# tum-vision/pnec

Hardware: AMD Instinct MI355X
Metric: PNEC pose solves/sec (512 corr, 10 GN iters) (higher is better)
Workload: dtype f64; 1 GPU; configs[1]: batch of 100k simulated frame pairs x 512 anisotropic-covariance correspondences per GPU; pairs_total=100000, launcher=single process, residual=PNEC target frame, setup_launches_before_warmup=15, pairs_per_gpu=100000, correspondences=512

## Files before the change

pnec_amd/csrc/pnec_solve_kernel.hpp:

```cpp
#pragma once

#include <type_traits>

#include "pnec_device.hpp"


#define PNEC_FOR_EACH_GEOMETRY(X) \
  X(1, 1, 0) X(2, 1, 0) X(4, 1, 0) X(4, 2, 0) X(4, 4, 0) X(4, 8, 0) \
  X(8, 1, 3) X(12, 1, 3) X(8, 2, 3) X(8, 4, 3) X(8, 8, 3) X(8, 1, 0) X(1, 8, 0)
#define PNEC_FOR_EACH_AOS_GEOMETRY(X) \
  X(1, 1, 0) X(2, 1, 0) X(4, 1, 0) X(4, 4, 0) X(4, 8, 0) X(8, 1, 3) X(8, 2, 3) X(8, 4, 3) X(8, 8, 3) X(8, 1, 0)
constexpr int kStreamWaves = 8;

namespace pnec_hip {

struct SolveArgs {
  const double *data;
  const int64_t *block_offset;
  const int32_t *count;
  const int32_t *pair_index;
  const double *init_q;
  const double *init_t;
  const double *hyp_t;
  double *out_q;
  double *out_t;
  double *out_cost;
  int32_t *out_iterations;
  int32_t *out_status;
  unsigned long long *trace;
  unsigned long long *work;
  int64_t n_solves;
  int32_t n_hyp;
  int32_t numeric_jacobian;
  const double *aos_bvs1, *aos_bvs2, *aos_covs, *aos_covs_host;
  const int64_t *aos_offsets;
  unsigned long long *done_counter;
  unsigned long long *host_flag;
  unsigned long long flag_value, n_blocks_total;
  double reg;
  double inv_max_radius;
  double inv_min_radius;
  pnec_hip_options opt;
};
inline void finish_args(SolveArgs &a) {
  a.inv_max_radius = 1.0 / a.opt.max_trust_region_radius;
  a.inv_min_radius = 1.0 / a.opt.min_trust_region_radius;
}

__device__ __forceinline__ int64_t xcd_contiguous_index(int64_t b, int64_t n) {
  const int64_t xcd = b & 7, q = n >> 3, r = n & 7;
  const int64_t base = (xcd < r) ? xcd * (q + 1) : r * (q + 1) + (xcd - r) * q;
  return base + (b >> 3);
}

enum : int {
  kQ = 0,
  kTheta = 4,
  kPhi = 5,
  kCost = 6,
  kXNorm = 7,
  kInvRadius = 8,
  kDec = 9,
  kModel = 10,
  kQc = 11,
  kThetaC = 15,
  kPhiC = 16,
  kDiag = 17,
  kScaleSq = 22,
  kInvScaleSq = 27,
  kGmax = 32,
  kSumsFinite = 33,
  kSums = 36,
  kTcur = 84,
  kSlab = 88
};
constexpr int kUnif = 18;
enum : int { kIIter = 0, kIFirst, kIReuseDiag, kINumInvalid, kIStepOk,
              kILast,
              kIPark,
              kITerm,
              kINumI = 8 };

__host__ __device__ constexpr bool geometry_ok(int mode, int cpl, int wpp, int ldsk) {
  const int nc = num_components(mode);
  if (cpl == 12) return wpp == 1 && ldsk == 3 && nc <= 12;
  const long lds = (long)wpp * (ldsk * nc * kWave * 8 + (kSlab + kUnif) * 8 + kINumI * 4) + (wpp > 1 ? 2L * wpp * kSumSlots * 8 : 0);
  if (lds > 160 * 1024) return false;
  if (cpl == 8 && ldsk == 0) return nc <= 18;
  return nc * (cpl - ldsk) <= 72;
}


__device__ __forceinline__ double atan2_c(double y, double x) {
  if (y == 0.0) return copysign(signbit(x) ? 3.14159265358979311600e+00 : 0.0, y);
  return atan2_lean(y, x);
}
__device__ __forceinline__ void start_angles(double x, double y, double z, double &theta, double &phi) {
  const double n = sqrt(x * x + y * y + z * z);
  if (n == 0.0) {
    theta = 0.0;
    phi = 0.0;
    return;
  }
  theta = acos_lean(z / n);
  phi = (fabs(theta) < 1e-10) ? 0.0 : atan2_c(y / n, x / n);
}

template <int CPL, int REGK>
__host__ __device__ constexpr int slot_corr(int k, int lane) {
  if (CPL == 1) return lane;
  if (k < (REGK & ~1)) return 2 * kWave * (k / 2) + 2 * lane + (k & 1);
  return kWave * k + lane;
}

template <int NC, int CPL, int REGK>
__device__ __forceinline__ void load_resident(const double *__restrict__ base, int n, int stride,
                                              int first_corr, int lane, double (&d)[REGK][NC],
                                              double *lds ) {
  (void)n;
  if constexpr (CPL == 1) {
    const int idx = first_corr + lane;
    const bool in = idx < stride;
#pragma unroll
    for (int c = 0; c < NC; ++c) d[0][c] = in ? base[(int64_t)c * stride + idx] : 0.0;
  } else {
    using pair_t = __attribute__((ext_vector_type(2))) double;
    auto load_pair = [&](auto jc) {
      constexpr int j = decltype(jc)::value;
      const int idx = first_corr + 2 * kWave * j + 2 * lane;
      const bool in = idx < stride;
#pragma unroll
      for (int c = 0; c < NC; ++c) {
        pair_t v = {0.0, 0.0};
        if (in) v = *reinterpret_cast<const pair_t *>(base + (int64_t)c * stride + idx);
        d[2 * j][c] = v.x;
        d[2 * j + 1][c] = v.y;
      }
    };
    if constexpr (REGK >= 2) load_pair(std::integral_constant<int, 0>{});
    if constexpr (REGK >= 4) load_pair(std::integral_constant<int, 1>{});
    if constexpr (REGK >= 6) load_pair(std::integral_constant<int, 2>{});
    if constexpr (REGK >= 8) load_pair(std::integral_constant<int, 3>{});
    if constexpr (REGK & 1) {
      const int idx = first_corr + kWave * (REGK - 1) + lane;
      const bool in = idx < stride;
#pragma unroll
      for (int c = 0; c < NC; ++c) d[REGK - 1][c] = in ? base[(int64_t)c * stride + idx] : 0.0;
    }
    typedef __attribute__((address_space(3))) void lds_void;
    typedef const __attribute__((address_space(1))) void global_void;
#pragma unroll
    for (int k = REGK; k < CPL; ++k) {
      const int chunk = first_corr + kWave * k;
      if (chunk < stride) {
        if (lane < kWave / 2) {
#pragma unroll
          for (int c = 0; c < NC; ++c)
            __builtin_amdgcn_global_load_lds((global_void *)(base + (int64_t)c * stride + chunk + 2 * lane),
                                             (lds_void *)(uintptr_t)(uint32_t)(uintptr_t)(lds + ((k - REGK) * NC + c) * kWave),
                                             16, 0, 0);
        }
      } else {
#pragma unroll
        for (int c = 0; c < NC; ++c) lds[((k - REGK) * NC + c) * kWave + lane] = 0.0;
      }
    }
  }
}

template <int NC, int CPL, int REGK>
__device__ __forceinline__ void load_resident_aos(const double *__restrict__ b1, const double *__restrict__ b2,
                                                  const double *__restrict__ cv, const double *__restrict__ ch,
                                                  int n, int first_corr, int lane, double (&d)[REGK][NC],
                                                  double *lds ) {
  auto put = [&](auto kc, int c, double v) {
    constexpr int k = decltype(kc)::value;
    if constexpr (k < REGK) d[k][c] = v;
    else lds[((k - REGK) * NC + c) * kWave + lane] = v;
  };
  auto load_slot = [&](auto kc) {
    constexpr int k = decltype(kc)::value;
    const int idx = first_corr + slot_corr<CPL, REGK>(k, lane);
    const bool in = idx < n;
    const int64_t j = in ? idx : 0;
#pragma unroll
    for (int c = 0; c < 3; ++c) {
      put(kc, c, in ? b1[3 * j + c] : 0.0);
      put(kc, 3 + c, in ? b2[3 * j + c] : 0.0);
    }
    if constexpr (NC >= 12) {
      const double *C = cv + 9 * j;
      put(kc, 6, in ? C[0] : 0.0);
      put(kc, 7, in ? 0.5 * (C[1] + C[3]) : 0.0);
      put(kc, 8, in ? 0.5 * (C[2] + C[6]) : 0.0);
      put(kc, 9, in ? C[4] : 0.0);
      put(kc, 10, in ? 0.5 * (C[5] + C[7]) : 0.0);
      put(kc, 11, in ? C[8] : 0.0);
    }
    if constexpr (NC >= 18) {
      const double *C = ch + 9 * j;
      put(kc, 12, in ? C[0] : 0.0);
      put(kc, 13, in ? 0.5 * (C[1] + C[3]) : 0.0);
      put(kc, 14, in ? 0.5 * (C[2] + C[6]) : 0.0);
      put(kc, 15, in ? C[4] : 0.0);
      put(kc, 16, in ? 0.5 * (C[5] + C[7]) : 0.0);
      put(kc, 17, in ? C[8] : 0.0);
    }
  };
  load_slot(std::integral_constant<int, 0>{});
  if constexpr (CPL >= 2) load_slot(std::integral_constant<int, 1>{});
  if constexpr (CPL >= 4) {
    load_slot(std::integral_constant<int, 2>{});
    load_slot(std::integral_constant<int, 3>{});
  }
  if constexpr (CPL >= 8) {
    load_slot(std::integral_constant<int, 4>{});
    load_slot(std::integral_constant<int, 5>{});
    load_slot(std::integral_constant<int, 6>{});
    load_slot(std::integral_constant<int, 7>{});
  }
}

template <int MODE, int REGK, int LDSK>
__device__ __forceinline__ void pass_resident(const double (&d)[REGK][num_components(MODE)],
                                              const double *lds , int nslots,
                                              int lane, const PassUniforms &U, double reg,
                                              double (&acc)[kNumAcc]) {
  constexpr int NC = num_components(MODE);
  auto eval_slot = [&](auto kc) {
    constexpr int k = decltype(kc)::value;
    double r, J[5];
    eval_corr<MODE>(d[k], U, reg, r, J);
    accumulate(r, J, acc);
  };
  eval_slot(std::integral_constant<int, 0>{});
  if constexpr (REGK > 1) eval_slot(std::integral_constant<int, 1>{});
  if constexpr (REGK > 2) {
    if (nslots > 2) {
      eval_slot(std::integral_constant<int, 2>{});
      if constexpr (REGK > 3) eval_slot(std::integral_constant<int, 3>{});
      if constexpr (REGK > 4) eval_slot(std::integral_constant<int, 4>{});
      if constexpr (REGK > 5) eval_slot(std::integral_constant<int, 5>{});
      if constexpr (REGK > 6) eval_slot(std::integral_constant<int, 6>{});
      if constexpr (REGK > 7) eval_slot(std::integral_constant<int, 7>{});
    }
  }
#pragma unroll
  for (int k = 0; k < LDSK; ++k) {
    if (REGK + k >= nslots) continue;
    double e[NC];
#pragma unroll
    for (int c = 0; c < NC; ++c) e[c] = lds[(k * NC + c) * kWave + lane];
    double r, J[5];
    eval_corr<MODE>(e, U, reg, r, J);
    accumulate(r, J, acc);
  }
}

template <int MODE, int REGK, int LDSK>
__device__ __forceinline__ void pass_cost_resident(const double (&d)[REGK][num_components(MODE)],
                                                   const double *lds , int nslots,
                                                   int lane, const PassUniforms &U, double reg,
                                                   double &acc0, double &z) {
  constexpr int NC = num_components(MODE);
  auto eval_slot = [&](auto kc) {
    constexpr int k = decltype(kc)::value;
    double r, kk;
    eval_cost<MODE>(d[k], U, reg, r, kk);
    acc0 = __builtin_fma(r, r, acc0);
    z = __builtin_fma(kk, 0.0, z);
  };
  eval_slot(std::integral_constant<int, 0>{});
  if constexpr (REGK > 1) eval_slot(std::integral_constant<int, 1>{});
  if constexpr (REGK > 2) {
    if (nslots > 2) {
      eval_slot(std::integral_constant<int, 2>{});
      if constexpr (REGK > 3) eval_slot(std::integral_constant<int, 3>{});
      if constexpr (REGK > 4) eval_slot(std::integral_constant<int, 4>{});
      if constexpr (REGK > 5) eval_slot(std::integral_constant<int, 5>{});
      if constexpr (REGK > 6) eval_slot(std::integral_constant<int, 6>{});
      if constexpr (REGK > 7) eval_slot(std::integral_constant<int, 7>{});
    }
  }
#pragma unroll
  for (int k = 0; k < LDSK; ++k) {
    if (REGK + k >= nslots) continue;
    double e[NC];
#pragma unroll
    for (int c = 0; c < NC; ++c) e[c] = lds[(k * NC + c) * kWave + lane];
    double r, kk;
    eval_cost<MODE>(e, U, reg, r, kk);
    acc0 = __builtin_fma(r, r, acc0);
    z = __builtin_fma(kk, 0.0, z);
  }
}

__device__ __forceinline__ void pose_uniforms_sc(double st, double ct, double sp, double cp, const double (&q)[4],
                                                 double *u) {
  double R[9];
  rot_from_quat(q, R);
#pragma unroll
  for (int i = 0; i < 9; ++i) u[i] = R[i];
  u[9] = st * cp;   u[10] = st * sp;  u[11] = ct;
  u[12] = ct * cp;  u[13] = ct * sp;  u[14] = -st;
}
__device__ __forceinline__ void pose_uniforms(double theta, double phi, const double (&q)[4], double *u) {
  double st, ct, sp, cp;
  sincos_bounded(theta, st, ct);
  sincos_bounded(phi, sp, cp);
  pose_uniforms_sc(st, ct, sp, cp, q, u);
}

__device__ __forceinline__ void write_result(const SolveArgs &a, int64_t s, const double *slab, int iteration,
                                             int term) {
  const double q0 = slab[kQ + 0], q1 = slab[kQ + 1], q2 = slab[kQ + 2], q3 = slab[kQ + 3];
  const double qn = fast_rsqrt(q0 * q0 + q1 * q1 + q2 * q2 + q3 * q3);
  if (a.out_q) {
    a.out_q[4 * s + 0] = q0 * qn;
    a.out_q[4 * s + 1] = q1 * qn;
    a.out_q[4 * s + 2] = q2 * qn;
    a.out_q[4 * s + 3] = q3 * qn;
  }
  if (a.out_t) {
    a.out_t[3 * s + 0] = slab[kTcur + 0];
    a.out_t[3 * s + 1] = slab[kTcur + 1];
    a.out_t[3 * s + 2] = slab[kTcur + 2];
  }
  if (a.out_cost) a.out_cost[s] = slab[kCost];
  if (a.out_iterations) a.out_iterations[s] = iteration;
  if (a.out_status) a.out_status[s] = term;
}

template <bool COST_FIRST>
__device__ __forceinline__ int lm_advance(double *slab, int *ist, double *unif, const pnec_hip_options &o,
                                          double inv_max_radius, double inv_min_radius) {
  int iteration = ist[kIIter], reuse_diagonal = ist[kIReuseDiag];
  int num_invalid = ist[kINumInvalid], step_ok = ist[kIStepOk];
  const int first = ist[kIFirst];
  const int pass_kind = ist[kILast];
  const bool last = pass_kind == 1;
  const bool cost_first = COST_FIRST && pass_kind == 2;
  int park = ist[kIPark];
  int term = -1;

  double S[kNumAcc];
  const double *cand_sums = slab + kSums + (park ^ 1) * kSumSlots;
#pragma unroll
  for (int j = 0; j < kNumAcc; ++j) S[j] = cand_sums[sum_slot(j)];
  const bool rest_ok = slab[kSumsFinite] != 0.0;
  const double qc0 = slab[kQc + 0], qc1 = slab[kQc + 1], qc2 = slab[kQc + 2], qc3 = slab[kQc + 3];
  const double thc0 = slab[kThetaC], phc0 = slab[kPhiC];
  const double cost = slab[kCost], model = slab[kModel], xnorm = slab[kXNorm];
  double inv_radius = slab[kInvRadius], dec = slab[kDec], gmax = slab[kGmax];
  double x[6];

  double cost_c = 0.5 * S[0];
  const bool cost_ok = finite_d(cost_c);
  bool accept = false;
  double rho = 0.0;
  if (first) {
    if (!(cost_ok && rest_ok)) {
      slab[kQ + 0] = qc0; slab[kQ + 1] = qc1; slab[kQ + 2] = qc2; slab[kQ + 3] = qc3;
      slab[kTheta] = thc0;
      slab[kPhi] = phc0;
        slab[kTcur + 0] = unif[9]; slab[kTcur + 1] = unif[10]; slab[kTcur + 2] = unif[11];
      slab[kCost] = cost_c;
      term = PNEC_HIP_TERM_BAD_INITIAL;
    } else {
#pragma unroll
      for (int i = 0; i < 5; ++i) {
        const double f = (i >= 2) ? 2.0 : 1.0, inv_f = (i >= 2) ? 0.5 : 1.0;
        const double hii = S[6 + tri(i, i)] * (f * f);
        const double a = (o.jacobi_scaling ? 1.0 + fast_sqrt(hii) : 1.0) * inv_f;
        slab[kInvScaleSq + i] = a * a;
        slab[kScaleSq + i] = fast_rcp(a * a);
      }
      accept = true;
    }
  } else {
    if (!cost_ok) cost_c = 1.7976931348623157e308;
    if (o.check_convergence) {
#pragma unroll
      for (int k = 0; k < 4; ++k) x[k] = slab[kQ + k];
      x[4] = slab[kTheta];
      x[5] = slab[kPhi];
      double dn = (x[4] - thc0) * (x[4] - thc0) + (x[5] - phc0) * (x[5] - phc0);
      dn = __builtin_fma(x[0] - qc0, x[0] - qc0, dn);
      dn = __builtin_fma(x[1] - qc1, x[1] - qc1, dn);
      dn = __builtin_fma(x[2] - qc2, x[2] - qc2, dn);
      dn = __builtin_fma(x[3] - qc3, x[3] - qc3, dn);
      const double step_norm = fast_sqrt(dn);
      if (step_norm <= o.parameter_tolerance * (xnorm + o.parameter_tolerance))
        term = PNEC_HIP_TERM_PARAMETER_TOL;
      else if (fabs(cost - cost_c) <= o.function_tolerance * cost)
        term = PNEC_HIP_TERM_FUNCTION_TOL;
    }
    if (term < 0) {
      rho = (cost - cost_c) * fast_rcp(model);
      accept = rho > o.min_relative_decrease;
      if (accept && !rest_ok) term = PNEC_HIP_TERM_BAD_INITIAL;
    }
  }

  if (term < 0 && cost_first && accept) {
    ist[kILast] = 0;
    return -1;
  }
  if (term < 0 && last) {
    if (accept) {
      slab[kQ + 0] = qc0; slab[kQ + 1] = qc1; slab[kQ + 2] = qc2; slab[kQ + 3] = qc3;
      slab[kTheta] = thc0;
      slab[kPhi] = phc0;
        slab[kTcur + 0] = unif[9]; slab[kTcur + 1] = unif[10]; slab[kTcur + 2] = unif[11];
      slab[kCost] = cost_c;
    }
    term = PNEC_HIP_TERM_MAX_ITERATIONS;
  }
  if (term < 0) {
    double H[15], g[5], diag[5];
    if (accept) {
      x[0] = qc0; x[1] = qc1; x[2] = qc2; x[3] = qc3; x[4] = thc0; x[5] = phc0;
#pragma unroll
      for (int i = 0; i < 5; ++i) g[i] = S[1 + i];
#pragma unroll
      for (int i = 0; i < 15; ++i) H[i] = S[6 + i];
      if (o.check_convergence) {
        gmax = 0.0;
#pragma unroll
        for (int i = 0; i < 5; ++i) gmax = fmax(gmax, fabs(g[i]) * ((i >= 2) ? 2.0 : 1.0));
      }
      if (first) {
        inv_radius = fast_rcp(o.initial_trust_region_radius);
      } else {
        const double c1 = 2.0 * rho - 1.0;
        inv_radius = fmax(inv_max_radius, inv_radius * fmax(1.0 / 3.0, 1.0 - c1 * c1 * c1));
      }
      dec = 2.0;
      park ^= 1;
      step_ok = 1;
      reuse_diagonal = 0;
#pragma unroll
      for (int k = 0; k < 4; ++k) slab[kQ + k] = x[k];
      slab[kTheta] = x[4];
      slab[kPhi] = x[5];
        slab[kTcur + 0] = unif[9]; slab[kTcur + 1] = unif[10]; slab[kTcur + 2] = unif[11];
      slab[kCost] = cost_c;
      if (o.check_convergence) {
        slab[kXNorm] = fast_sqrt(x[4] * x[4] + x[5] * x[5] + x[0] * x[0] + x[1] * x[1] + x[2] * x[2] + x[3] * x[3]);
        slab[kGmax] = gmax;
      }
    } else {
#pragma unroll
      for (int k = 0; k < 4; ++k) x[k] = slab[kQ + k];
      x[4] = slab[kTheta];
      x[5] = slab[kPhi];
      const double *cur_sums = slab + kSums + park * kSumSlots;
#pragma unroll
      for (int i = 0; i < 5; ++i) g[i] = cur_sums[sum_slot(1 + i)];
#pragma unroll
      for (int i = 0; i < 15; ++i) H[i] = cur_sums[sum_slot(6 + i)];
      inv_radius = inv_radius * dec;
      dec = 2.0 * dec;
      reuse_diagonal = 1;
    }
    if (reuse_diagonal) {
#pragma unroll
      for (int i = 0; i < 5; ++i) diag[i] = slab[kDiag + i];
    }

    for (bool retry = false;; retry = true) {
      if (iteration >= o.max_num_iterations) { term = PNEC_HIP_TERM_MAX_ITERATIONS; break; }
      if (retry) {
        const double *cur_sums = slab + kSums + park * kSumSlots;
#pragma unroll
        for (int i = 0; i < 15; ++i) H[i] = cur_sums[sum_slot(6 + i)];
      }
      if (o.check_convergence && step_ok && gmax <= o.gradient_tolerance) {
        term = PNEC_HIP_TERM_GRADIENT_TOL; break;
      }
      if (inv_radius > inv_min_radius) { term = PNEC_HIP_TERM_MIN_RADIUS; break; }
      ++iteration;
      step_ok = 0;

      if (!reuse_diagonal) {
#pragma unroll
        for (int i = 0; i < 5; ++i) {
          diag[i] = fmin(fmax(H[tri(i, i)] * slab[kScaleSq + i], o.min_lm_diagonal), o.max_lm_diagonal) *
                    slab[kInvScaleSq + i];
          slab[kDiag + i] = diag[i];
        }
      }
      double dr[5], y[5], step[5];
#pragma unroll
      for (int i = 0; i < 5; ++i) {
        dr[i] = diag[i] * inv_radius;
        H[tri(i, i)] += dr[i];
      }
      bool valid = chol_solve5(H, g, y);
      double sg = 0.0, sd = 0.0;
#pragma unroll
      for (int i = 0; i < 5; ++i) {
        step[i] = -y[i];
        sg = __builtin_fma(step[i], g[i], sg);
        sd = __builtin_fma(dr[i] * step[i], step[i], sd);
      }
      const double model_change = 0.5 * (sd - sg);
      valid = valid && (model_change > 0.0);
      if (!valid) {
        if (++num_invalid >= o.max_num_consecutive_invalid_steps) { term = PNEC_HIP_TERM_INVALID_STEPS; break; }
        inv_radius = 2.0 * inv_radius;
        reuse_diagonal = 1;
        continue;
      }
      num_invalid = 0;

      const double dx = 0.5 * step[2], dy = 0.5 * step[3], dz = 0.5 * step[4];
      const double thc = x[4] + step[0];
      const double phc = x[5] + step[1];
      const double nd2 = dx * dx + dy * dy + dz * dz;
      const double ind = nd2 > 0.0 ? fast_rsqrt(nd2) : 0.0, nd = nd2 * ind;
      const int role = (int)(threadIdx.x & 3);
      const double angle = role == 0 ? nd : (role == 1 ? thc : phc);
      double sa, ca;
      sincos_bounded_pinned(angle, sa, ca);
      const double sn = quad_broadcast<0>(sa), aw = quad_broadcast<0>(ca);
      const double st = quad_broadcast<1>(sa), ct = quad_broadcast<1>(ca);
      const double sp = quad_broadcast<2>(sa), cp = quad_broadcast<2>(ca);
      const double sbd = sn * ind;
      const double ax = sbd * dx, ay = sbd * dy, az = sbd * dz;
      double qc[4];
      qc[0] = aw * x[0] + ax * x[3] + ay * x[2] - az * x[1];
      qc[1] = aw * x[1] - ax * x[2] + ay * x[3] + az * x[0];
      qc[2] = aw * x[2] + ax * x[1] - ay * x[0] + az * x[3];
      qc[3] = aw * x[3] - ax * x[0] - ay * x[1] - az * x[2];
      pose_uniforms_sc(st, ct, sp, cp, qc, unif);
#pragma unroll
      for (int k = 0; k < 4; ++k) slab[kQc + k] = qc[k];
      slab[kThetaC] = thc;
      slab[kPhiC] = phc;
      slab[kModel] = model_change;
      const double cost_now = accept ? cost_c : cost;
      ist[kILast] = iteration >= o.max_num_iterations ? 1 : ((COST_FIRST && (!accept || model_change <= 4.0e-15 * cost_now)) ? 2 : 0);
      break;
    }
    slab[kInvRadius] = inv_radius;
    slab[kDec] = dec;
  }
  ist[kIPark] = park;

  ist[kIIter] = iteration;
  ist[kIFirst] = (term < 0 || !first) ? 0 : 1;
  ist[kIReuseDiag] = reuse_diagonal;
  ist[kINumInvalid] = num_invalid;
  ist[kIStepOk] = step_ok;
  return term;
}

constexpr int kNumPoses = 12;
__device__ __forceinline__ void numeric_poses(const double *slab, int lane, double (*nu)[12], double *inv2h) {
  if (lane < kNumPoses) {
    const int prm = lane >> 1;
    double x[6] = {slab[kThetaC], slab[kPhiC], slab[kQc + 0], slab[kQc + 1], slab[kQc + 2], slab[kQc + 3]};
    const double xv = prm == 0 ? x[0] : (prm == 1 ? x[1] : (prm == 2 ? x[2] : (prm == 3 ? x[3] : (prm == 4 ? x[4] : x[5]))));
    const double h = fmax(1.4901161193847656e-08, fabs(xv) * 1e-6);
    const double xp = (lane & 1) ? xv - h : xv + h;
#pragma unroll
    for (int k = 0; k < 6; ++k) x[k] = (k == prm) ? xp : x[k];
    double u[kUnif];
    const double q[4] = {x[2], x[3], x[4], x[5]};
    pose_uniforms(x[0], x[1], q, u);
#pragma unroll
    for (int i = 0; i < 12; ++i) nu[lane][i] = u[i];
    if ((lane & 1) == 0) inv2h[prm] = 1.0 / h / 2.0;
  }
}
template <int MODE>
__device__ __forceinline__ void eval_corr_numeric(const double (&e)[num_components(MODE)], const PassUniforms &U,
                                                  const double (*nu)[12], const double *inv2h, const double *qc,
                                                  double reg, double &r, double (&J)[5]) {
  double kk;
  eval_cost<MODE>(e, U, reg, r, kk);
  double Ja[6];
#pragma unroll 1
  for (int prm = 0; prm < 6; ++prm) {
    double rr[2];
#pragma unroll
    for (int sgn = 0; sgn < 2; ++sgn) {
      PassUniforms V;
      const double *u = nu[2 * prm + sgn];
#pragma unroll
      for (int i = 0; i < 9; ++i) V.R[i] = u[i];
#pragma unroll
      for (int i = 0; i < 3; ++i) V.t[i] = u[9 + i];
      eval_cost<MODE>(e, V, reg, rr[sgn], kk);
    }
    Ja[prm] = (rr[0] - rr[1]) * inv2h[prm];
  }
  J[0] = Ja[0];
  J[1] = Ja[1];
  const double qx = qc[0], qy = qc[1], qz = qc[2], qw = qc[3];
  J[2] = 0.5 * (Ja[2] * qw + Ja[3] * -qz + Ja[4] * qy + Ja[5] * -qx);
  J[3] = 0.5 * (Ja[2] * qz + Ja[3] * qw + Ja[4] * -qx + Ja[5] * -qy);
  J[4] = 0.5 * (Ja[2] * -qy + Ja[3] * qx + Ja[4] * qw + Ja[5] * -qz);
}

#ifdef PNEC_ISA_MARKS
#define PNEC_MARK(name) asm volatile("; PNEC_MARK " name)
#else
#define PNEC_MARK(name)
#endif

constexpr int SRC_PLANES = 0;
constexpr int SRC_AOS = 1;
template <int MODE, int CPL, int WPP, int LDSK, bool RESIDENT, int SRC = SRC_PLANES>
__global__ __launch_bounds__(kWave *WPP, (CPL == 8 && LDSK == 0) ? 1 : 2) void lm_solve_kernel(const SolveArgs a) {
  static_assert(SRC != SRC_AOS || RESIDENT, "the AoS source is only built for the on-chip-resident geometries");
  constexpr int NC = num_components(MODE);
  constexpr int RCPL = CPL > 8 ? 8 : CPL;
  constexpr int TAILK = CPL - RCPL;
  static_assert(TAILK == 0 || (TAILK == 4 && WPP == 1 && RESIDENT && SRC != SRC_AOS), "the tail form is (12, 1, 3) on the batch's planes");
  constexpr int REGK = RESIDENT ? RCPL - LDSK : 1;
  const int lane = threadIdx.x & (kWave - 1);
  const int wave = threadIdx.x >> 6;
  const int64_t slot = xcd_contiguous_index(blockIdx.x, a.n_solves);
  const int64_t pair = a.pair_index ? (int64_t)a.pair_index[slot / a.n_hyp] : slot / a.n_hyp;
  const int64_t s = pair * a.n_hyp + slot % a.n_hyp;
  const double *__restrict__ base = nullptr;
  int n;
  int64_t aos0 = 0;
  if constexpr (SRC == SRC_AOS) {
    aos0 = a.aos_offsets[pair];
    n = (int)(a.aos_offsets[pair + 1] - aos0);
  } else {
    base = a.data + a.block_offset[pair];
    n = a.count[pair];
  }
  const int stride = (n + kWave - 1) & ~(kWave - 1);
  const pnec_hip_options &o = a.opt;
  const double reg = a.reg;

  unsigned long long t_begin = 0, t_loaded = 0;
  if (a.trace) t_begin = __builtin_amdgcn_s_memtime();

  __shared__ double slab_all[WPP][kSlab];
  __shared__ double unif_all[WPP][kUnif];
  __shared__ int ist_all[WPP][kINumI];
  [[maybe_unused]] __shared__ double xw[2][WPP > 1 ? WPP : 1][kSumSlots];
  [[maybe_unused]] __shared__ double nunif[RESIDENT ? 1 : kNumPoses][12];
  [[maybe_unused]] __shared__ double ninv2h[8];
  [[maybe_unused]] __shared__ double ldata[LDSK > 0 ? WPP : 1][LDSK > 0 ? LDSK : 1][NC][LDSK > 0 ? kWave : 1];
  double *slab = slab_all[WPP > 1 ? 0 : wave];
  double *unif = unif_all[WPP > 1 ? 0 : wave];
  int *ist = ist_all[WPP > 1 ? 0 : wave];
  [[maybe_unused]] int parity = 0;

  double d[REGK][NC];
  if constexpr (RESIDENT && SRC == SRC_AOS)
    load_resident_aos<NC, RCPL, REGK>(a.aos_bvs1 + 3 * aos0, a.aos_bvs2 + 3 * aos0, NC >= 12 ? a.aos_covs + 9 * aos0 : nullptr,
                                     NC >= 18 ? a.aos_covs_host + 9 * aos0 : nullptr, n, wave * RCPL * kWave, lane, d,
                                     &ldata[LDSK > 0 ? wave : 0][0][0][0]);
  else if constexpr (RESIDENT)
    load_resident<NC, RCPL, REGK>(base, n, stride, wave * RCPL * kWave, lane, d, &ldata[LDSK > 0 ? wave : 0][0][0][0]);
  [[maybe_unused]] int nslots = 0;
  if constexpr (RESIDENT) {
#pragma unroll
    for (int k = 0; k < RCPL; ++k) nslots += (n > wave * RCPL * kWave + slot_corr<RCPL, REGK>(k, 0)) ? 1 : 0;
  }
  [[maybe_unused]] int ntail = 0;
  [[maybe_unused]] const char *tail_base = nullptr;
  [[maybe_unused]] size_t tail_plane_bytes = 0;
  if constexpr (TAILK > 0) {
#pragma unroll
    for (int t = 0; t < TAILK; ++t) ntail += (n > RCPL * kWave + 2 * kWave * (t / 2) + (t & 1)) ? 1 : 0;
    const unsigned long long b64 = reinterpret_cast<unsigned long long>(base) + (unsigned long long)RCPL * kWave * sizeof(double);
    const unsigned blo = (unsigned)__builtin_amdgcn_readfirstlane((int)(unsigned)b64);
    const unsigned bhi = (unsigned)__builtin_amdgcn_readfirstlane((int)(unsigned)(b64 >> 32));
    tail_base = reinterpret_cast<const char *>(((unsigned long long)bhi << 32) | blo);
    tail_plane_bytes = (size_t)(unsigned)__builtin_amdgcn_readfirstlane(stride) * sizeof(double);
    ntail = __builtin_amdgcn_readfirstlane(ntail);
  }
  if (a.trace) {
    __builtin_amdgcn_s_waitcnt(0);
    t_loaded = __builtin_amdgcn_s_memtime();
  }

  if (lane == 0 && (WPP == 1 || wave == 0)) {
    double th, ph;
    const double *t0 = a.hyp_t ? a.hyp_t + 3 * s : a.init_t + 3 * pair;
    start_angles(t0[0], t0[1], t0[2], th, ph);
    double q[4];
#pragma unroll
    for (int k = 0; k < 4; ++k) {
      q[k] = a.init_q[pair * 4 + k];
      slab[kQc + k] = q[k];
    }
    slab[kThetaC] = th;
    slab[kPhiC] = ph;
    pose_uniforms(th, ph, q, unif);
    ist[kIIter] = 0;
    ist[kIFirst] = 1;
    ist[kIReuseDiag] = 0;
    ist[kINumInvalid] = 0;
    ist[kIStepOk] = 1;
    ist[kILast] = o.max_num_iterations <= 0 ? 1 : 0;
    ist[kIPark] = 0;
  }
  const double inv_max_radius = a.inv_max_radius, inv_min_radius = a.inv_min_radius;
  if constexpr (RESIDENT && LDSK > 0 && SRC != SRC_AOS) __builtin_amdgcn_s_waitcnt(0x0F70);
  __builtin_amdgcn_fence(__ATOMIC_RELEASE, "wavefront");
  if constexpr (WPP > 1) __syncthreads();

  int term;
  int n_full_passes = 0, n_cost_passes = 0;
  for (;;) {
    PNEC_MARK("uniforms");
    {
      __builtin_amdgcn_fence(__ATOMIC_ACQUIRE, "wavefront");
      PassUniforms U;
#pragma unroll
      for (int i = 0; i < 9; ++i) U.R[i] = to_sgpr(unif[i]);
#pragma unroll
      for (int i = 0; i < 3; ++i) U.t[i] = to_sgpr(unif[9 + i]);
#pragma unroll
      for (int i = 0; i < 3; ++i) U.bth[i] = to_sgpr(unif[12 + i]);
      U.bph[0] = -U.t[1];
      U.bph[1] = U.t[0];
      U.bph[2] = 0.0;
      double c[6];
      bool cost_only = false;
      if constexpr (RESIDENT) cost_only = to_sgpr(ist[kILast]) != 0;
      n_cost_passes += cost_only ? 1 : 0;
      n_full_passes += cost_only ? 0 : 1;
      if (cost_only) {
        PNEC_MARK("pass_cost");
        if constexpr (RESIDENT) {
          double a0 = 0.0, z = 0.0;
          pass_cost_resident<MODE, REGK, LDSK>(d, &ldata[LDSK > 0 ? wave : 0][0][0][0], nslots, lane, U, reg,
                                               a0, z);
          c[0] = wave_reduce_acc0_row0(a0);
          c[1] = __builtin_amdgcn_ballot_w64(!(z == 0.0)) == 0ull ? 0.0 : __builtin_nan("");
          c[2] = c[3] = c[4] = c[5] = 0.0;
          if constexpr (TAILK > 0) {
            if (ntail > 0) {
              double a1 = 0.0, z1 = 0.0;
              const char *tb = tail_base;
              const size_t plane_bytes = tail_plane_bytes;
              const unsigned voff = 16u * (unsigned)lane;
              auto tail_cost = [&](auto tc) {
                constexpr int t = decltype(tc)::value;
                constexpr unsigned imm = 2u * kWave * 8u * (t / 2) + 8u * (t & 1);
                const bool in = RCPL * kWave + 2 * kWave * (t / 2) + 2 * lane < stride;
                double e[NC];
                load_planes_saddr<NC, (int)imm>(e, tb, plane_bytes, voff, in);
                double r, kk;
                eval_cost<MODE>(e, U, reg, r, kk);
                a1 = __builtin_fma(r, r, a1);
                z1 = __builtin_fma(kk, 0.0, z1);
              };
              tail_cost(std::integral_constant<int, 0>{});
              __builtin_amdgcn_sched_barrier(0);
              tail_cost(std::integral_constant<int, 1>{});
              __builtin_amdgcn_sched_barrier(0);
              if (ntail > 2) {
                tail_cost(std::integral_constant<int, 2>{});
                __builtin_amdgcn_sched_barrier(0);
                tail_cost(std::integral_constant<int, 3>{});
                __builtin_amdgcn_sched_barrier(0);
              }
              c[0] += wave_reduce_acc0_row0(a1);
              c[1] += __builtin_amdgcn_ballot_w64(!(z1 == 0.0)) == 0ull ? 0.0 : __builtin_nan("");
            }
          }
        }
      } else {
        double acc[kNumAcc];
#pragma unroll
        for (int j = 0; j < kNumAcc; ++j) acc[j] = 0.0;
        PNEC_MARK("pass");
        if constexpr (RESIDENT) {
          pass_resident<MODE, REGK, LDSK>(d, &ldata[LDSK > 0 ? wave : 0][0][0][0], nslots, lane, U, reg, acc);
        } else {
          const bool numeric = a.numeric_jacobian != 0;
          if (numeric) {
            if (wave == 0) numeric_poses(slab, lane, nunif, ninv2h);
            __syncthreads();
          }
          for (int idx = threadIdx.x; idx < stride; idx += kWave * WPP) {
            double e[NC];
#pragma unroll
            for (int c = 0; c < NC; ++c) e[c] = base[(int64_t)c * stride + idx];
            double r, J[5];
            if (numeric) eval_corr_numeric<MODE>(e, U, nunif, ninv2h, slab + kQc, reg, r, J);
            else eval_corr<MODE>(e, U, reg, r, J);
            accumulate(r, J, acc);
          }
        }
        PNEC_MARK("reduce");
        wave_reduce21_rows(acc, c);
        if constexpr (TAILK > 0) {
          if (ntail > 0) {
            double *park_sums = slab + kSums + (to_sgpr(ist[kIPark]) ^ 1) * kSumSlots;
            if ((lane & 15) == 0) {
#pragma unroll
              for (int i = 0; i < 6; ++i) park_sums[(lane >> 4) * 6 + i] = c[i];
            }
#pragma unroll
            for (int j = 0; j < kNumAcc; ++j) acc[j] = 0.0;
            const char *tb = tail_base;
            const size_t plane_bytes = tail_plane_bytes;
            const unsigned voff = 16u * (unsigned)lane;
            auto tail_slot = [&](auto tc) {
              constexpr int t = decltype(tc)::value;
              constexpr unsigned imm = 2u * kWave * 8u * (t / 2) + 8u * (t & 1);
              const bool in = RCPL * kWave + 2 * kWave * (t / 2) + 2 * lane < stride;
              double e[NC];
              load_planes_saddr<NC, (int)imm>(e, tb, plane_bytes, voff, in);
              double r, J[5];
              eval_corr<MODE>(e, U, reg, r, J);
              accumulate(r, J, acc);
            };
            tail_slot(std::integral_constant<int, 0>{});
            __builtin_amdgcn_sched_barrier(0);
            tail_slot(std::integral_constant<int, 1>{});
            __builtin_amdgcn_sched_barrier(0);
            if (ntail > 2) {
              tail_slot(std::integral_constant<int, 2>{});
              __builtin_amdgcn_sched_barrier(0);
              tail_slot(std::integral_constant<int, 3>{});
              __builtin_amdgcn_sched_barrier(0);
            }
            double c2[6];
            wave_reduce21_rows(acc, c2);
            __builtin_amdgcn_fence(__ATOMIC_RELEASE, "wavefront");
            __builtin_amdgcn_wave_barrier();
            __builtin_amdgcn_fence(__ATOMIC_ACQUIRE, "wavefront");
#pragma unroll
            for (int i = 0; i < 6; ++i) c[i] = park_sums[(lane >> 4) * 6 + i] + c2[i];
          }
        }
      }
      double *cand_sums = slab + kSums + (to_sgpr(ist[kIPark]) ^ 1) * kSumSlots;
      if constexpr (WPP == 1) {
        const bool fin = rows_all_finite(c);
        if ((lane & 15) == 0) {
#pragma unroll
          for (int i = 0; i < 6; ++i) cand_sums[(lane >> 4) * 6 + i] = c[i];
          if (lane == 0) slab[kSumsFinite] = fin ? 1.0 : 0.0;
        }
      } else {
        if ((lane & 15) == 0) {
#pragma unroll
          for (int i = 0; i < 6; ++i) xw[parity][wave][(lane >> 4) * 6 + i] = c[i];
        }
        __syncthreads();
        if (wave == 0 && lane == 0) {
          double z = 0.0;
#pragma unroll
          for (int j = 0; j < kSumSlots; ++j) {
            double t = xw[parity][0][j];
#pragma unroll
            for (int w = 1; w < WPP; ++w) t += xw[parity][w][j];
            cand_sums[j] = t;
            z = __builtin_fma(t, 0.0, z);
          }
          slab[kSumsFinite] = (z == 0.0) ? 1.0 : 0.0;
        }
        parity ^= 1;
      }
    }

    PNEC_MARK("advance");
    __builtin_amdgcn_fence(__ATOMIC_RELEASE, "wavefront");
    int t = -1;
    if constexpr (WPP == 1) {
      __builtin_amdgcn_s_setprio(3);
      if (lane < 4) t = lm_advance<RESIDENT>(slab, ist, unif, o, inv_max_radius, inv_min_radius);
      term = to_sgpr(t);
      __builtin_amdgcn_s_setprio(0);
      __builtin_amdgcn_fence(__ATOMIC_RELEASE, "wavefront");
    } else {
      if (wave == 0) {
        __builtin_amdgcn_s_setprio(3);
        if (lane < 4) t = lm_advance<RESIDENT>(slab, ist, unif, o, inv_max_radius, inv_min_radius);
        if (lane == 0) ist[kITerm] = t;
        __builtin_amdgcn_s_setprio(0);
      }
      __syncthreads();
      term = to_sgpr(ist[kITerm]);
    }
    if (term >= 0) break;
  }

  PNEC_MARK("result");
  if (threadIdx.x == 0) {
    write_result(a, s, slab, ist[kIIter], term);
    if (a.work) {
      atomicAdd(a.work + 0, (unsigned long long)n_full_passes * (unsigned long long)n);
      atomicAdd(a.work + 1, (unsigned long long)n_cost_passes * (unsigned long long)n);
    }
    if constexpr (SRC == SRC_AOS) {
      __threadfence_system();
      const unsigned long long done = atomicAdd(a.done_counter, 1ull) + 1ull;
      if (done == a.n_blocks_total) {
        __hip_atomic_store(a.host_flag, a.flag_value, __ATOMIC_RELEASE, __HIP_MEMORY_SCOPE_SYSTEM);
      }
    }
    if (a.trace && threadIdx.x == 0) {
      unsigned hw = 0;
      asm volatile("s_getreg_b32 %0, hwreg(HW_REG_HW_ID)" : "=s"(hw));
      unsigned xcc = 0;
      asm volatile("s_getreg_b32 %0, hwreg(HW_REG_XCC_ID)" : "=s"(xcc));
      a.trace[4 * (size_t)blockIdx.x + 0] = t_begin;
      a.trace[4 * (size_t)blockIdx.x + 1] = t_loaded;
      a.trace[4 * (size_t)blockIdx.x + 2] = __builtin_amdgcn_s_memtime();
      a.trace[4 * (size_t)blockIdx.x + 3] = ((unsigned long long)xcc << 32) | hw;
    }
  }
}

}
```

Before: 36.78 million solves/s.

## Speculate rejected-step fallback candidates in spare lanes and specialize the residual Jacobian

In single-wave resident geometries, three extra lane quads now solve the damped system at successively larger damping while the primary quad solves the normal step. The fallback candidates are staged in LDS, so a rejected step can take the next candidate directly and skip a re-solve in the serial Levenberg-Marquardt advance. A hand-written residual and Jacobian routine for the NEC and target modes replaces the generic eval_corr in the solve passes to cut arithmetic per correspondence. In exchange the change adds LDS usage, extra lanes in the advance step, and extra control logic, and it can only help when steps are actually rejected.

```diff
diff --git a/pnec_amd/csrc/pnec_solve_kernel.hpp b/pnec_amd/csrc/pnec_solve_kernel.hpp
--- a/pnec_amd/csrc/pnec_solve_kernel.hpp
+++ b/pnec_amd/csrc/pnec_solve_kernel.hpp
@@ -79,12 +79,17 @@
               kILast,
               kIPark,
               kITerm,
+              kISpec = kITerm,
               kINumI = 8 };
+constexpr int kNumFallbacks = 3;
+enum : int { kSpModel = 0, kSpQc = 1, kSpThetaC = 5, kSpPhiC = 6, kSpValid = 7, kSpUnif = 8 , kSpecSlot = 24 };
+static_assert(kQc - kModel == kSpQc && kThetaC - kModel == kSpThetaC && kPhiC - kModel == kSpPhiC, "slot layout = slab layout");
 
 __host__ __device__ constexpr bool geometry_ok(int mode, int cpl, int wpp, int ldsk) {
   const int nc = num_components(mode);
   if (cpl == 12) return wpp == 1 && ldsk == 3 && nc <= 12;
-  const long lds = (long)wpp * (ldsk * nc * kWave * 8 + (kSlab + kUnif) * 8 + kINumI * 4) + (wpp > 1 ? 2L * wpp * kSumSlots * 8 : 0);
+  const long lds = (long)wpp * (ldsk * nc * kWave * 8 + (kSlab + kUnif) * 8 + kINumI * 4) + (wpp > 1 ? 2L * wpp * kSumSlots * 8 : 0) +
+                   (wpp == 1 ? kNumFallbacks * kSpecSlot * 8 : 0);
   if (lds > 160 * 1024) return false;
   if (cpl == 8 && ldsk == 0) return nc <= 18;
   return nc * (cpl - ldsk) <= 72;
@@ -221,6 +226,52 @@
   }
 }
 
+template <int MODE>
+__device__ __forceinline__ void eval_corr_solve(const double (&d)[num_components(MODE)], const PassUniforms &U,
+                                                double reg, double &r, double (&J)[5]) {
+  if constexpr (MODE != PNEC_HIP_MODE_NEC && MODE != PNEC_HIP_MODE_TARGET) {
+    eval_corr<MODE>(d, U, reg, r, J);
+  } else {
+    const double f1x = d[0], f1y = d[1], f1z = d[2];
+    const double f2x = d[3], f2y = d[4], f2z = d[5];
+    const double *R = U.R;
+    const double mx = U.t[1] * f1z - U.t[2] * f1y;
+    const double my = U.t[2] * f1x - U.t[0] * f1z;
+    const double mz = U.t[0] * f1y - U.t[1] * f1x;
+    const double gx = R[0] * mx + R[3] * my + R[6] * mz;
+    const double gy = R[1] * mx + R[4] * my + R[7] * mz;
+    const double gz = R[2] * mx + R[5] * my + R[8] * mz;
+    const double n = f2x * gx + f2y * gy + f2z * gz;
+    double wx, wy, wz;
+    if constexpr (MODE == PNEC_HIP_MODE_NEC) {
+      r = n;
+      wx = f2x; wy = f2y; wz = f2z;
+    } else {
+      const double sgx = d[6] * gx + d[7] * gy + d[8] * gz;
+      const double sgy = d[7] * gx + d[9] * gy + d[10] * gz;
+      const double sgz = d[8] * gx + d[10] * gy + d[11] * gz;
+      const double den = gx * sgx + gy * sgy + gz * sgz + reg;
+      const double y = fast_rsqrt(fmax(den, kTinyDen));
+      r = n * y;
+      const double c = r * y;
+      wx = y * (f2x - c * sgx);
+      wy = y * (f2y - c * sgy);
+      wz = y * (f2z - c * sgz);
+    }
+    const double ux = R[0] * wx + R[1] * wy + R[2] * wz;
+    const double uy = R[3] * wx + R[4] * wy + R[5] * wz;
+    const double uz = R[6] * wx + R[7] * wy + R[8] * wz;
+    J[2] = __builtin_fma(uy, mz, -(uz * my));
+    J[3] = __builtin_fma(uz, mx, -(ux * mz));
+    J[4] = __builtin_fma(ux, my, -(uy * mx));
+    const double jx = __builtin_fma(f1y, uz, -(f1z * uy));
+    const double jy = __builtin_fma(f1z, ux, -(f1x * uz));
+    const double jz = __builtin_fma(f1x, uy, -(f1y * ux));
+    J[0] = U.bth[0] * jx + U.bth[1] * jy + U.bth[2] * jz;
+    J[1] = U.bph[0] * jx + U.bph[1] * jy;
+  }
+}
+
 template <int MODE, int REGK, int LDSK>
 __device__ __forceinline__ void pass_resident(const double (&d)[REGK][num_components(MODE)],
                                               const double *lds , int nslots,
@@ -230,7 +281,7 @@
   auto eval_slot = [&](auto kc) {
     constexpr int k = decltype(kc)::value;
     double r, J[5];
-    eval_corr<MODE>(d[k], U, reg, r, J);
+    eval_corr_solve<MODE>(d[k], U, reg, r, J);
     accumulate(r, J, acc);
   };
   eval_slot(std::integral_constant<int, 0>{});
@@ -252,7 +303,7 @@
 #pragma unroll
     for (int c = 0; c < NC; ++c) e[c] = lds[(k * NC + c) * kWave + lane];
     double r, J[5];
-    eval_corr<MODE>(e, U, reg, r, J);
+    eval_corr_solve<MODE>(e, U, reg, r, J);
     accumulate(r, J, acc);
   }
 }
@@ -331,9 +382,14 @@
   if (a.out_status) a.out_status[s] = term;
 }
 
-template <bool COST_FIRST>
+template <bool COST_FIRST, int NFB = 0>
 __device__ __forceinline__ int lm_advance(double *slab, int *ist, double *unif, const pnec_hip_options &o,
-                                          double inv_max_radius, double inv_min_radius) {
+                                          double inv_max_radius, double inv_min_radius,
+                                          [[maybe_unused]] double *spec = nullptr ) {
+  static_assert(NFB == 0 || NFB == kNumFallbacks, "one quad per fallback: lanes 4 .. 15");
+  [[maybe_unused]] const int quad = NFB > 0 ? (int)((threadIdx.x >> 2) & 3) : 0;
+  [[maybe_unused]] int served = 0;
+  if constexpr (NFB > 0) served = ist[kISpec];
   int iteration = ist[kIIter], reuse_diagonal = ist[kIReuseDiag];
   int num_invalid = ist[kINumInvalid], step_ok = ist[kIStepOk];
   const int first = ist[kIFirst];
@@ -406,6 +462,30 @@
     ist[kILast] = 0;
     return -1;
   }
+  if constexpr (NFB > 0) {
+    if (term < 0 && !last && !accept && served < NFB && iteration < o.max_num_iterations) {
+      const double *slot = spec + served * kSpecSlot;
+      if (slot[kSpValid] != 0.0) {
+        inv_radius = inv_radius * dec;
+        dec = 2.0 * dec;
+        ++iteration;
+#pragma unroll
+        for (int k = 0; k < kSpValid; ++k) slab[kModel + k] = slot[k];
+#pragma unroll
+        for (int i = 0; i < 15; ++i) unif[i] = slot[kSpUnif + i];
+        slab[kInvRadius] = inv_radius;
+        slab[kDec] = dec;
+        ist[kILast] = iteration >= o.max_num_iterations ? 1 : (COST_FIRST ? 2 : 0);
+        ist[kISpec] = served + 1;
+        ist[kIIter] = iteration;
+        ist[kIFirst] = 0;
+        ist[kIReuseDiag] = 1;
+        ist[kINumInvalid] = 0;
+        ist[kIStepOk] = 0;
+        return -1;
+      }
+    }
+  }
   if (term < 0 && last) {
     if (accept) {
       slab[kQ + 0] = qc0; slab[kQ + 1] = qc1; slab[kQ + 2] = qc2; slab[kQ + 3] = qc3;
@@ -490,10 +570,19 @@
           slab[kDiag + i] = diag[i];
         }
       }
+      double ir = inv_radius;
+      if constexpr (NFB > 0) {
+        double fd = dec;
+#pragma unroll
+        for (int k = 0; k < NFB; ++k) {
+          ir = k < quad ? ir * fd : ir;
+          fd = 2.0 * fd;
+        }
+      }
       double dr[5], y[5], step[5];
 #pragma unroll
       for (int i = 0; i < 5; ++i) {
-        dr[i] = diag[i] * inv_radius;
+        dr[i] = diag[i] * ir;
         H[tri(i, i)] += dr[i];
       }
       bool valid = chol_solve5(H, g, y);
@@ -506,7 +595,15 @@
       }
       const double model_change = 0.5 * (sd - sg);
       valid = valid && (model_change > 0.0);
-      if (!valid) {
+      if constexpr (NFB > 0) {
+        const bool primary_ok = (__builtin_amdgcn_ballot_w64(valid) & 1ull) != 0ull;
+        if (quad > 0) {
+          const bool ok = valid && primary_ok && !(ir > inv_min_radius);
+          spec[(quad - 1) * kSpecSlot + kSpValid] = ok ? 1.0 : 0.0;
+          if (!ok) break;
+        }
+      }
+      if ((NFB == 0 || quad == 0) && !valid) {
         if (++num_invalid >= o.max_num_consecutive_invalid_steps) { term = PNEC_HIP_TERM_INVALID_STEPS; break; }
         inv_radius = 2.0 * inv_radius;
         reuse_diagonal = 1;
@@ -533,15 +630,28 @@
       qc[1] = aw * x[1] - ax * x[2] + ay * x[3] + az * x[0];
       qc[2] = aw * x[2] + ax * x[1] - ay * x[0] + az * x[3];
       qc[3] = aw * x[3] - ax * x[0] - ay * x[1] - az * x[2];
-      pose_uniforms_sc(st, ct, sp, cp, qc, unif);
-#pragma unroll
-      for (int k = 0; k < 4; ++k) slab[kQc + k] = qc[k];
-      slab[kThetaC] = thc;
-      slab[kPhiC] = phc;
-      slab[kModel] = model_change;
+      double *cand_out = slab + kModel, *unif_out = unif;
+      if constexpr (NFB > 0) {
+        if (quad > 0) {
+          cand_out = spec + (quad - 1) * kSpecSlot;
+          unif_out = cand_out + kSpUnif;
+        }
+      }
+      pose_uniforms_sc(st, ct, sp, cp, qc, unif_out);
+#pragma unroll
+      for (int k = 0; k < 4; ++k) cand_out[kSpQc + k] = qc[k];
+      cand_out[kSpThetaC] = thc;
+      cand_out[kSpPhiC] = phc;
+      cand_out[kSpModel] = model_change;
       const double cost_now = accept ? cost_c : cost;
-      ist[kILast] = iteration >= o.max_num_iterations ? 1 : ((COST_FIRST && (!accept || model_change <= 4.0e-15 * cost_now)) ? 2 : 0);
+      if (NFB == 0 || quad == 0) {
+        ist[kILast] = iteration >= o.max_num_iterations ? 1 : ((COST_FIRST && (!accept || model_change <= 4.0e-15 * cost_now)) ? 2 : 0);
+        if constexpr (NFB > 0) ist[kISpec] = 0;
+      }
       break;
+    }
+    if constexpr (NFB > 0) {
+      if (quad > 0) return -1;
     }
     slab[kInvRadius] = inv_radius;
     slab[kDec] = dec;
@@ -645,6 +755,8 @@
   __shared__ double slab_all[WPP][kSlab];
   __shared__ double unif_all[WPP][kUnif];
   __shared__ int ist_all[WPP][kINumI];
+  constexpr int NFB = (WPP == 1 && RESIDENT && CPL == 8 && LDSK == 3) ? kNumFallbacks : 0;
+  [[maybe_unused]] __shared__ double spec_all[NFB > 0 ? WPP : 1][NFB > 0 ? NFB * kSpecSlot : 1];
   [[maybe_unused]] __shared__ double xw[2][WPP > 1 ? WPP : 1][kSumSlots];
   [[maybe_unused]] __shared__ double nunif[RESIDENT ? 1 : kNumPoses][12];
   [[maybe_unused]] __shared__ double ninv2h[8];
@@ -704,6 +816,7 @@
     ist[kIStepOk] = 1;
     ist[kILast] = o.max_num_iterations <= 0 ? 1 : 0;
     ist[kIPark] = 0;
+    if constexpr (WPP == 1) ist[kISpec] = kNumFallbacks;
   }
   const double inv_max_radius = a.inv_max_radius, inv_min_radius = a.inv_min_radius;
   if constexpr (RESIDENT && LDSK > 0 && SRC != SRC_AOS) __builtin_amdgcn_s_waitcnt(0x0F70);
@@ -791,7 +904,7 @@
             for (int c = 0; c < NC; ++c) e[c] = base[(int64_t)c * stride + idx];
             double r, J[5];
             if (numeric) eval_corr_numeric<MODE>(e, U, nunif, ninv2h, slab + kQc, reg, r, J);
-            else eval_corr<MODE>(e, U, reg, r, J);
+            else eval_corr_solve<MODE>(e, U, reg, r, J);
             accumulate(r, J, acc);
           }
         }
@@ -816,7 +929,7 @@
               double e[NC];
               load_planes_saddr<NC, (int)imm>(e, tb, plane_bytes, voff, in);
               double r, J[5];
-              eval_corr<MODE>(e, U, reg, r, J);
+              eval_corr_solve<MODE>(e, U, reg, r, J);
               accumulate(r, J, acc);
             };
             tail_slot(std::integral_constant<int, 0>{});
@@ -874,7 +987,7 @@
     int t = -1;
     if constexpr (WPP == 1) {
       __builtin_amdgcn_s_setprio(3);
-      if (lane < 4) t = lm_advance<RESIDENT>(slab, ist, unif, o, inv_max_radius, inv_min_radius);
+      if (lane < 4 * (1 + NFB)) t = lm_advance<RESIDENT, NFB>(slab, ist, unif, o, inv_max_radius, inv_min_radius, spec_all[NFB > 0 ? wave : 0]);
       term = to_sgpr(t);
       __builtin_amdgcn_s_setprio(0);
       __builtin_amdgcn_fence(__ATOMIC_RELEASE, "wavefront");
```

After: 38.01 million solves/s, median of 6. +3.4%, better.
